# jdeschut/tunempc

Measured on AMD Instinct MI355X. Metric: stage-Hessian convexifications/sec at (nx+nu)=32, p=64, higher is better.
Workload: dtype f64

## Files before the change

### tunempc_amd/csrc/tmpc_persist.h

```cpp
#pragma once
#include "tmpc_common.h"
#include "tmpc_cr_small.h"
#include "tmpc_factor.h"
#include "tmpc_schur.h"
#include "tmpc_stage.h"

namespace tmpc {

constexpr int PK_NMAX = sm8::NMAX;
constexpr int PK_WAVE_DOUBLES = 6 * sm8::MS + 16;
static_assert(PK_WAVE_DOUBLES >= sm8::MS + 160, "step-length scratch");
static_assert(PK_WAVE_DOUBLES >= 25 * 10 + 16, "records of schur_body<0> at nx = 5");
constexpr int pk_lds_doubles(int p) {
  int v = CRS_NW * PK_WAVE_DOUBLES;
  if (crs_factor_lds_doubles() > v) v = crs_factor_lds_doubles();
  if (crs_solve_lds_doubles(p) > v) v = crs_solve_lds_doubles(p);
  return v;
}

__global__ void __launch_bounds__(CRS_NT) k_ipm_small(WS w, Dims dm, Opts o, CrDev cr, CrLevs lv, int prep, int reg_max, double chord_pre, int cap) {
  extern __shared__ __attribute__((aligned(16))) double lds[];
  const int b = w.alist ? w.alist[blockIdx.x] : (int)blockIdx.x;
  const int tid = threadIdx.x, lane = tid & 63, wv = tid >> 6;
  double* smw = lds + wv * PK_WAVE_DOUBLES;
  const int p = dm.p, s0 = b * p;
  volatile int* ip = w.iprob + (size_t)b * IS;
#ifdef TMPC_CYCLE_PROF
  unsigned long long tpk_ = __builtin_readcyclecounter();
#define PK_T(i) { __syncthreads(); if (blockIdx.x == 0 && threadIdx.x == 0) { const unsigned long long t_ = __builtin_readcyclecounter(); g_prof[48 + (i)] += t_ - tpk_; tpk_ = t_; } }
#else
#define PK_T(i) __syncthreads();
#endif
  for (int it = 0; it < cap; ++it) {
    if (ip[I_PHASE] == PH_DONE) break;
    for (int k = wv; k < p; k += CRS_NW) sm8::stage_pre_body<64>(w, dm, s0 + k, lane, smw);
    PK_T(0)
    if (wv == 0) ctrl_a_body(w, dm, o, b, lane);
    PK_T(1)
    const int phase = ip[I_PHASE];
    if (phase == PH_DONE) break;
    if (!ip[I_CHORD]) {
      for (int k = wv; k < p; k += CRS_NW) {
        schur_body<0, false, 64>(w, dm, s0 + k, lane, smw);
        schur_body<1, false, 64>(w, dm, s0 + k, lane, smw);
      }
      PK_T(2)
      if (prep) { cr_prep_body<CRS_NT>(w, dm, b, prep); __syncthreads(); }
      cr_small_factor_body(w, dm, cr, lv, b, lds);
      PK_T(3)
    }
    for (int pass = 1; pass <= 2; ++pass) {
      if (pass == 2 || phase == PH_MAIN) {
        for (int k = wv; k < p; k += CRS_NW) sm8::stage_rhs_body<64>(w, dm, s0 + k, lane, smw, pass);
        PK_T(4)
        for (int k = wv; k < p; k += CRS_NW) gather_body(w, dm, s0 + k, lane, pass);
        PK_T(5)
        cr_small_solve_body(w, dm, cr, lv, b, lds, pass);
        PK_T(6)
        solve_border_body<CRS_NT>(w, dm, b, pass, lds);
        PK_T(7)
        for (int k = wv; k < p; k += CRS_NW) sm8::stage_dir_body<64>(w, dm, s0 + k, lane, smw, pass);
        PK_T(8)
        for (int m = tid; m < 4 * p; m += CRS_NT) eigmin_lane_body(w, dm, 4 * s0 + m, pass);
        PK_T(9)
      }
      if (wv == 0) { if (pass == 1) ctrl_b_body(w, dm, reg_max, b, lane); else ctrl_c_body(w, dm, reg_max, b, lane); }
      PK_T(10)
    }
    for (int k = wv; k < p; k += CRS_NW) sm8::update_body<64>(w, dm, s0 + k, lane);
    __syncthreads();
    if (tid == 0) ctrl_d_body(w, dm, o, b, false);
    PK_T(11)
  }
#undef PK_T
}

}
```

### tunempc_amd/csrc/tmpc_stage.h

```cpp
#pragma once
#include "tmpc_common.h"
#include "tmpc_small.h"

namespace tmpc {

__device__ __forceinline__ int stage_id4(const WS& w, const Dims& dm) {
  if (!w.alist) return blockIdx.x;
  const int sb = blockIdx.x >> 2, bi = sb / dm.p;
  return ((w.alist[bi] * dm.p + (sb - bi * dm.p)) << 2) | (blockIdx.x & 3);
}

#define TMPC_STAGE_PROLOGUE                                     \
  const int sid = stage_id(w, dm);                              \
  const int b = sid / dm.p;                                     \
  const int k = sid - b * dm.p;                                 \
  const int lane = threadIdx.x;                                 \
  const int n = dm.n, nx = dm.nx;                               \
  const int nn = n * n, nxx = nx * nx;                          \
  (void)k; (void)nn; (void)nxx;                                 \
  extern __shared__ __attribute__((aligned(16))) double sm[];

#ifdef TMPC_EIG_DEBUG
__device__ int g_eig_dbg[4]; __device__ double g_eig_dbgv[8];
#endif

__device__ __forceinline__ int stage_rows(const WS& w, const Dims& dm, size_t sid) {
  int nc = w.ncnt ? w.ncnt[sid] : 0;
  nc = nc < 0 ? 0 : (nc > dm.nr - dm.ng ? dm.nr - dm.ng : nc);
  return dm.ng + nc;
}

#include "tmpc_stage_impl.h"
namespace sm8 {
#include "tmpc_stage_impl.h"
}

__global__ void __launch_bounds__(64) k_init_stage(WS w, Dims dm) {
  TMPC_STAGE_PROLOGUE
  double* sH = sm; double* cs = sm + MS;
  const double* Hg = w.H + (size_t)sid * nn;
  for (int e = lane; e < nn; e += 64) {
    int i, j; ediv(e, n, i, j);
    sH[i * LD + j] = 0.5 * (Hg[i * n + j] + Hg[j * n + i]);
  }
  wsync();
  s2g(w.Hb + (size_t)sid * nn, sH, n, n, n, lane);
  jacobi_eigvals(sH, n, cs, lane);
  double lo = 1e300, hi = -1e300, amin = 1e300, amax = 0.0;
  if (lane < n) {
    const double ev = sH[lane * LD + lane];
    lo = ev; hi = ev;
    const double a = fabs(ev);
    if (a != 0.0) { amin = a; amax = a; }
  }
  lo = wave_min(lo); hi = wave_max(hi); amin = wave_min(amin); amax = wave_max(amax);
  if (lane == 0) {
    double* q = w.part + (size_t)sid * NPART;
    q[Q_MINEIG] = lo; q[Q_MAXEIG] = hi; q[Q_MINABS] = amin; q[Q_MAXABS] = amax;
  }
  const int mb = dm.mb;
  double* Vg = w.V + (size_t)sid * nx * n;
  const double* Ag = w.A + (size_t)sid * nxx;
  const double* Bg = w.Bm + (size_t)sid * nx * mb;
  for (int e = lane; e < nx * n; e += 64) {
    int i, j; ediv(e, n, i, j);
    Vg[e] = (j < nx) ? Ag[i * nx + j] : Bg[i * mb + (j - nx)];
  }
}

__global__ void __launch_bounds__(64) k_init_prob(WS w, Dims dm, double lowp_switch) {
  const int b = blockIdx.x, lane = threadIdx.x;
  double lo = 1e300, amin = 1e10 , amax = 0.0;
  for (int k = lane; k < dm.p; k += 64) {
    const double* q = w.part + (size_t)(b * dm.p + k) * NPART;
    lo = fmin(lo, q[Q_MINEIG]); amin = fmin(amin, q[Q_MINABS]); amax = fmax(amax, q[Q_MAXABS]);
  }
  lo = wave_min(lo); amin = wave_min(amin); amax = wave_max(amax);
  if (lane == 0) {
    double* pr = w.prob + (size_t)b * PS;
    int* ip = w.iprob + (size_t)b * IS;
    for (int i = 0; i < PS; ++i) pr[i] = 0.0;
    for (int i = 0; i < IS; ++i) ip[i] = 0;
    const double s = 1.0 / amin, sbeta = amax / amin;
    pr[P_S] = s; pr[P_SBETA] = sbeta; pr[P_MINEIG_H] = lo;
    pr[P_TAU] = 2.0; pr[P_ALPHA] = 1.0 / sbeta; pr[P_S0] = 1.0 / sbeta; pr[P_X0] = 1.0 / (double)(dm.p * dm.n);
    pr[P_MUT] = -1.0; pr[P_PREVSTEPN] = -1.0; pr[P_STEPN] = 1e300; pr[P_MINPIV] = 1.0;
    const int early = (lo > 0.0) ? 1 : 0;
    ip[I_EARLY] = early;
    ip[I_PHASE] = early ? PH_DONE : PH_MAIN;
    ip[I_IPMSTATUS] = early ? IPM_OPTIMAL : IPM_MAXITER;
    if (!early) { const int slot = atomicAdd(w.active, 1); w.alist[slot] = b; w.flist[slot] = b; }
    if (!early && (dm.flags & DF_LOWP) && w.O32 && 2.0 / (double)(2 * dm.p * dm.n + 1) > lowp_switch * fmax(1.0, fabs(pr[P_TAU]))) { ip[I_LOWP] = 1; atomicAdd(w.active + 4, 1); }
  }
}

__global__ void __launch_bounds__(64) k_init_state(WS w, Dims dm) {
  TMPC_STAGE_PROLOGUE
  const double* pr = w.prob + (size_t)b * PS;
  const double s = pr[P_S], tau = pr[P_TAU], alpha = pr[P_ALPHA];
  const double x0 = 1.0 / (double)(dm.p * n);
  double* Hb = w.Hb + (size_t)sid * nn;
  for (int e = lane; e < nn; e += 64) {
    int i, j; ediv(e, n, i, j);
    const double hb = s * Hb[e];
    Hb[e] = hb;
    const double dg = (i == j) ? 1.0 : 0.0;
    w.S1[(size_t)sid * nn + e] = dg;
    w.S2[(size_t)sid * nn + e] = tau * dg - alpha * hb;
    w.X1[(size_t)sid * nn + e] = x0 * dg;
    w.X2[(size_t)sid * nn + e] = x0 * dg;
  }
  for (int e = lane; e < nxx; e += 64) w.P[(size_t)sid * nxx + e] = 0.0;
}

__device__ __forceinline__ double lane_min_eig8(const double* __restrict__ Wg, int n) {
  double a[36];
#define TMPC_A8(i, j) a[(i) * ((i) + 1) / 2 + (j)]
#define TMPC_S8(r, c) (((c) <= (r)) ? TMPC_A8(r, c) : TMPC_A8(c, r))
#pragma unroll
  for (int i = 0; i < 8; ++i)
#pragma unroll
    for (int j = 0; j <= i; ++j) TMPC_A8(i, j) = (i < n) ? 0.5 * (Wg[i * n + j] + Wg[j * n + i]) : 0.0;
#pragma unroll
  for (int j = 0; j < 6; ++j) {
    double sigma = 0.0;
#pragma unroll
    for (int i = j + 2; i < 8; ++i) sigma = fma(TMPC_A8(i, j), TMPC_A8(i, j), sigma);
    if (sigma != 0.0) {
      const double x0 = TMPC_A8(j + 1, j);
      const double mu = sqrt(fma(x0, x0, sigma));
      const double v0 = (x0 <= 0.0) ? (x0 - mu) : (-sigma / (x0 + mu));
      const double beta = 2.0 * v0 * v0 / (sigma + v0 * v0);
      const double rv0 = 1.0 / v0;
      double v[8], pw[8];
#pragma unroll
      for (int i = j + 1; i < 8; ++i) v[i] = (i == j + 1) ? 1.0 : TMPC_A8(i, j) * rv0;
      double kk = 0.0;
#pragma unroll
      for (int r = j + 1; r < 8; ++r) {
        double acc = 0.0;
#pragma unroll
        for (int c = j + 1; c < 8; ++c) acc = fma(TMPC_S8(r, c), v[c], acc);
        pw[r] = beta * acc;
        kk = fma(pw[r], v[r], kk);
      }
      kk *= 0.5 * beta;
#pragma unroll
      for (int r = j + 1; r < 8; ++r) pw[r] = fma(-kk, v[r], pw[r]);
#pragma unroll
      for (int r = j + 1; r < 8; ++r)
#pragma unroll
        for (int c = j + 1; c <= r; ++c) TMPC_A8(r, c) -= fma(v[r], pw[c], pw[r] * v[c]);
      TMPC_A8(j + 1, j) = mu;
    }
  }
  double dd[8], ee[8];
#pragma unroll
  for (int i = 0; i < 8; ++i) { dd[i] = TMPC_A8(i, i); ee[i] = (i < 7) ? TMPC_A8(i + 1, i) : 0.0; }
#undef TMPC_S8
#undef TMPC_A8
  if (n == 1) return dd[0];
  double scale = 0.0;
  bool bad = false;
#pragma unroll
  for (int i = 0; i < 8; ++i) if (i < n) { bad |= !(dd[i] == dd[i]) || ((i + 1 < n) && !(ee[i] == ee[i])); scale = fmax(scale, fmax(fabs(dd[i]), (i + 1 < n) ? fabs(ee[i]) : 0.0)); }
  if (bad) return __builtin_nan("");
  if (!(scale > 0.0) || !(scale < 1e300)) return (scale == 0.0) ? 0.0 : scale;
  const double rs = 1.0 / scale;
  double e2[8];
  double lo = 1e300;
#pragma unroll
  for (int i = 0; i < 8; ++i) {
    dd[i] *= rs; ee[i] *= rs; e2[i] = ee[i] * ee[i];
  }
#pragma unroll
  for (int i = 0; i < 8; ++i)
    if (i < n) lo = fmin(lo, dd[i] - ((i > 0) ? fabs(ee[i - 1]) : 0.0) - ((i + 1 < n) ? fabs(ee[i]) : 0.0));
  double x = lo - 1e-14;
  const double dn = (double)n;
  for (int it = 0; it < 64; ++it) {
    double qm = 1.0, q = dd[0] - x, gm = 0.0, g = -1.0, hm = 0.0, h = 0.0;
#pragma unroll
    for (int i = 1; i < 8; ++i) {
      if (i < n) {
        const double t = dd[i] - x, c = e2[i - 1];
        const double qn = fma(t, q, -c * qm);
        const double gn = fma(t, g, -c * gm) - q;
        const double hn = fma(t, h, -c * hm) - 2.0 * g;
        qm = q; q = qn; gm = g; g = gn; hm = h; h = hn;
      }
    }
    if (!(q > 0.0)) break;
    const double G = g / q, H = G * G - h / q;
    double disc = (dn - 1.0) * (dn * H - G * G);
    if (!(disc > 0.0)) disc = 0.0;
    const double step = dn / (sqrt(disc) - G);
    if (!(step > 4e-16 * fmax(1.0, fabs(x)))) break;
    x += step;
  }
  return x * scale;
}
__device__ __forceinline__ void eigmin_lane_body(const WS& w, const Dims& dm, int mid, int pass) {
  const int b = (mid >> 2) / dm.p;
  const int phase = w.iprob[(size_t)b * IS + I_PHASE];
  if (phase == PH_DONE || (pass == 1 && phase != PH_MAIN)) return;
  w.eigmin[mid] = lane_min_eig8(w.Wm + (size_t)mid * dm.n * dm.n, dm.n);
}
__global__ void __launch_bounds__(64) k_eigmin_lane(WS w, Dims dm, int pass, int nmat) {
  const int i = blockIdx.x * 64 + threadIdx.x;
  if (i >= nmat) return;
  const int sb = i >> 2, bi = sb / dm.p;
  const int mid = w.alist ? (((w.alist[bi] * dm.p + (sb - bi * dm.p)) << 2) | (i & 3)) : i;
  eigmin_lane_body(w, dm, mid, pass);
}

template <int NT>
__global__ void __launch_bounds__(NT, NT == 256 ? 3 : 1) k_stage_pre(WS w, Dims dm) {
  extern __shared__ __attribute__((aligned(16))) double sm[];
  stage_pre_body<NT>(w, dm, stage_id(w, dm), threadIdx.x, sm);
}
template <int NT>
__global__ void __launch_bounds__(NT, NT == 256 ? 3 : 1) k_stage_rhs(WS w, Dims dm, int pass) {
  extern __shared__ __attribute__((aligned(16))) double sm[];
  stage_rhs_body<NT>(w, dm, stage_id(w, dm), threadIdx.x, sm, pass);
}
template <int NT>
__global__ void __launch_bounds__(NT, NT == 256 ? 3 : 1) k_stage_dir(WS w, Dims dm, int pass) {
  extern __shared__ __attribute__((aligned(16))) double sm[];
  stage_dir_body<NT>(w, dm, stage_id(w, dm), threadIdx.x, sm, pass);
}
__global__ void __launch_bounds__(64) k_eigmin(WS w, Dims dm, int pass, double chord_step) {
  extern __shared__ __attribute__((aligned(16))) double sm[];
  eigmin_body(w, dm, stage_id4(w, dm), threadIdx.x, sm, pass, chord_step);
}
template <int NT>
__global__ void __launch_bounds__(NT) k_update(WS w, Dims dm) {
  update_body<NT>(w, dm, stage_id(w, dm), threadIdx.x);
}

constexpr int FIN_SLOTS = 6;
__global__ void __launch_bounds__(64) k_final_stage(WS w, Dims dm) {
  TMPC_STAGE_PROLOGUE
  const int* ip = w.iprob + (size_t)b * IS;
  const double* pr = w.prob + (size_t)b * PS;
  double* sV = sm; double* sM = sm + MS; double* t0 = sm + 2 * MS; double* t1 = sm + 3 * MS; double* sHb = sm + 4 * MS;
  double* cs = sm + 5 * MS;
  const int kn = (k + 1 == dm.p) ? 0 : k + 1;
  const double sc = ip[I_EARLY] ? 0.0 : 1.0 / (pr[P_S] * pr[P_ALPHA]);
  double* Po = w.Pout + (size_t)sid * nxx;
  for (int e = lane; e < nxx; e += 64) Po[e] = sc * w.P[(size_t)sid * nxx + e];
  double* Pon = w.Pout + (size_t)(b * dm.p + kn) * nxx;
  const double* Pn = w.P + (size_t)(b * dm.p + kn) * nxx;
  if (kn != k) { for (int e = lane; e < nxx; e += 64) Pon[e] = sc * Pn[e]; }
  __threadfence_block();
  wsync();
  g2s(sV, w.V + (size_t)sid * nx * n, nx, n, n, lane);
  const double* Hg = w.H + (size_t)sid * nn;
  for (int e = lane; e < nn; e += 64) { int i, j; ediv(e, n, i, j); sHb[i * LD + j] = 0.5 * (Hg[i * n + j] + Hg[j * n + i]); }
  wsync();
  build_M(sM, sV, t0, t1, sHb, Po, Pon, 0.0, n, nx, lane);
  if (dm.nr > 0) {
    const int nrow = stage_rows(w, dm, sid);
    if (lane < dm.nr) w.Fg[(size_t)sid * dm.nr + lane] = (lane < nrow) ? sc * w.phi[(size_t)sid * dm.nr + lane] : 0.0;
    add_gtg(sM, w.G + (size_t)sid * dm.nr * n, w.phi + (size_t)sid * dm.nr, sc, nrow, n, lane);
  }
  if (dm.nT > 0) {
    add_smat_t3(sM, w.t3th + (size_t)sid * dm.nT, sc, n, lane);
    for (int e = lane; e < nn; e += 64) {
      int i, j; ediv(e, n, i, j);
      const int a = i < j ? i : j, bq = i < j ? j : i;
      w.Tout[(size_t)sid * nn + e] = sc * w.t3th[(size_t)sid * dm.nT + a * n - a * (a - 1) / 2 + (bq - a)];
    }
  }
  s_sym(sM, n, lane);
  double* dHg = w.dHc + (size_t)sid * nn;
  double* Hcg = w.Hc + (size_t)sid * nn;
  for (int e = lane; e < nn; e += 64) {
    int i, j; ediv(e, n, i, j);
    const double dh = sM[i * LD + j];
    dHg[e] = dh;
    const double hc = sHb[i * LD + j] + dh;
    Hcg[e] = hc;
    t0[i * LD + j] = hc;
  }
  wsync();
  const double lo = tridiag_min_eig(t0, n, cs, lane);
  const double hi = tridiag_max_after(cs, n, lane);
  if (lane == 0) {
    double* q = w.part + (size_t)sid * NPART;
    q[Q_MINEIG] = lo; q[Q_MAXEIG] = hi;
  }
}

__global__ void __launch_bounds__(64) k_final_prob(WS w, Dims dm) {
  const int b = blockIdx.x, lane = threadIdx.x;
  double lo = 1e300, hi = -1e300, mc = 0.0;
  for (int k = lane; k < dm.p; k += 64) {
    const double* q = w.part + (size_t)(b * dm.p + k) * NPART;
    lo = fmin(lo, q[Q_MINEIG]); hi = fmax(hi, q[Q_MAXEIG]);
    mc = fmax(mc, (q[Q_MINEIG] > 0.0) ? q[Q_MAXEIG] / q[Q_MINEIG] : 1e300);
  }
  lo = wave_min(lo); hi = wave_max(hi); mc = wave_max(mc);
  if (lane == 0) {
    double* pr = w.prob + (size_t)b * PS;
    int* ip = w.iprob + (size_t)b * IS;
    pr[P_MINEIG_HC] = lo; pr[P_MAXEIG_HC] = hi; pr[P_MAXCOND] = mc;
    int st;
    if (lo > 0.0) st = (ip[I_IPMSTATUS] == IPM_OPTIMAL || ip[I_IPMSTATUS] == IPM_FAST_EXIT || ip[I_IPMSTATUS] == IPM_TIGHT_FALLBACK) ? ST_OPTIMAL : ST_FEASIBLE;
    else st = ST_INFEASIBLE;
    ip[I_STATUS] = st;
    if (ip[I_EARLY]) { pr[P_KAPPA] = 0.0; pr[P_BETA] = 0.0; pr[P_ALPHA_OUT] = 1.0; }
    else { pr[P_KAPPA] = pr[P_TAU]; pr[P_BETA] = pr[P_TAU] / pr[P_SBETA]; pr[P_ALPHA_OUT] = pr[P_ALPHA]; }
  }
}

}
```

### tunempc_amd/csrc/tmpc_stage_impl.h

```cpp
template <int NT = 64>
__device__ __forceinline__ void s2g_T(double* g, const double* s, int rows, int cols, int ldg, int lane) {
  const int tot = rows * cols;
  for (int e = lane; e < tot; e += NT) {
    const int j = e / rows, i = e - j * rows;
    g[(size_t)j * ldg + i] = s[i * LD + j];
  }
  wsync();
}

template <int NT = 64>
__device__ __forceinline__ void build_M(double* out, const double* sV, double* t0, double* t1, const double* sHb,
                                        const double* Pk, const double* Pn, double coef, int n, int nx, int lane) {
  g2s<NT>(t0, Pn, nx, nx, nx, lane);
  mm<NT>(t1, sV, 1, LD, t0, LD, 1, n, nx, nx, 0, lane);
  mm<NT>(out, t1, LD, 1, sV, LD, 1, n, n, nx, 0, lane);
  g2s<NT>(t0, Pk, nx, nx, nx, lane);
  for (int e = lane; e < n * n; e += NT) {
    int i, j; ediv(e, n, i, j);
    double v = out[i * LD + j] + coef * sHb[i * LD + j];
    if (i < nx && j < nx) v -= t0[i * LD + j];
    out[i * LD + j] = v;
  }
  wsync();
}

template <int NT = 64>
__device__ __forceinline__ void adj_V(double* out, double* t, const double* sV, const double* G, int n, int nx, int lane) {
  mm<NT>(t, sV, LD, 1, G, LD, 1, nx, n, n, 0, lane);
  mm<NT>(out, t, LD, 1, sV, 1, LD, nx, nx, n, 0, lane);
}

template <int NT = 64>
__device__ __forceinline__ void add_gtg(double* out, const double* Gg, const double* coef, double scale, int ng, int n, int lane) {
  for (int e = lane; e < n * n; e += NT) {
    int i, j; ediv(e, n, i, j);
    double acc = 0.0;
    for (int r = 0; r < ng; ++r) acc = fma(scale * coef[r] * Gg[r * n + i], Gg[r * n + j], acc);
    out[i * LD + j] += acc;
  }
  wsync();
}

template <int NT = 64>
__device__ __forceinline__ void add_smat_t3(double* out, const double* th, double scale, int n, int lane) {
  for (int e = lane; e < n * n; e += NT) {
    int i, j; ediv(e, n, i, j);
    const int a = i < j ? i : j, b = i < j ? j : i;
    out[i * LD + j] += scale * th[a * n - a * (a - 1) / 2 + (b - a)];
  }
  wsync();
}

constexpr int PRE_SLOTS = 6;
template <int NT>
__device__ __forceinline__ void stage_pre_body(const WS& w, const Dims& dm, int sid, int lane, double* sm) {
  const int b = sid / dm.p;
  const int k = sid - b * dm.p;
  const int n = dm.n, nx = dm.nx;
  const int nn = n * n, nxx = nx * nx;
  (void)k; (void)nn; (void)nxx;
  const int* ip = w.iprob + (size_t)b * IS;
  if (ip[I_PHASE] == PH_DONE) return;
  const double* pr = w.prob + (size_t)b * PS;
  const double alpha = pr[P_ALPHA], tau = pr[P_TAU];
  double* sV = sm; double* sX = sm + MS; double* sS = sm + 2 * MS; double* t0 = sm + 3 * MS; double* t1 = sm + 4 * MS; double* sLi = sm + 5 * MS;
  double* sHb = sX;
  double* sM = sS;
  double* sSi = sS;
  double* t2 = sLi;
  double* sPhi = sX;
  constexpr int EPT = NMAX * NMAX / NT;
  double hbr[EPT], phir[EPT];
  const int kn = (k + 1 == dm.p) ? 0 : k + 1;
  TMPC_T0()
  double ldA[EPT];
  g2r<NT>(ldA, w.V + (size_t)sid * nx * n, nx, n, n, lane);
  g2r<NT>(hbr, w.Hb + (size_t)sid * nn, n, n, n, lane);
  r2s<NT>(sV, ldA, nx, n, lane);
  r2s<NT>(sHb, hbr, n, n, lane);
  TMPC_T(8)
#pragma unroll
  for (int q = 0; q < EPT; ++q) phir[q] = 0.0;
  build_M<NT>(sM, sV, t0, t1, sHb, w.P + (size_t)sid * nxx, w.P + (size_t)(b * dm.p + kn) * nxx, alpha, n, nx, lane);
  if (dm.nr > 0) add_gtg<NT>(sM, w.G + (size_t)sid * dm.nr * n, w.phi + (size_t)sid * dm.nr, 1.0, stage_rows(w, dm, sid), n, lane);
  if (dm.nT > 0) add_smat_t3<NT>(sM, w.t3th + (size_t)sid * dm.nT, 1.0, n, lane);
  TMPC_T(9)
  double rd2 = 0.0, s2 = 0.0, xs = 0.0, trx2 = 0.0, hby = 0.0, trpsi = 0.0, trphi2 = 0.0;
  int nbad = 0;
  double* kf = w.KF + (size_t)sid * 12 * nxx;
  for (int r = 0; r < 2; ++r) {
    const double* Sg = (r ? w.S2 : w.S1) + (size_t)sid * nn;
    double* Rdg = (r ? w.Rd2 : w.Rd1) + (size_t)sid * nn;
    for (int e = lane; e < nn; e += NT) {
      int i, j; ediv(e, n, i, j);
      const double m = sM[i * LD + j], sv = Sg[e];
      const double dg = (i == j) ? 1.0 : 0.0;
      const double rd = (r == 0 ? (m - dg) : (tau * dg - m)) - sv;
      Rdg[e] = rd;
      rd2 = fma(rd, rd, rd2); s2 = fma(sv, sv, s2);
    }
  }
  wsync();
  TMPC_T(10)
  for (int r = 0; r < 2; ++r) {
    const double* Xg = (r ? w.X2 : w.X1) + (size_t)sid * nn;
    const double* Sg = (r ? w.S2 : w.S1) + (size_t)sid * nn;
    {
      double ldB[EPT];
      g2r<NT>(ldA, Xg, n, n, n, lane);
      g2r<NT>(ldB, Sg, n, n, n, lane);
      r2s<NT>(sX, ldA, n, n, lane);
      r2s<NT>(sS, ldB, n, n, lane);
    }
    TMPC_T(8)
    for (int e = lane; e < nn; e += NT) { int i, j; ediv(e, n, i, j); xs = fma(sX[i * LD + j], sS[i * LD + j], xs); }
    {
      double hx = 0.0;
#pragma unroll
      for (int q = 0; q < EPT; ++q) { const int e = lane + q * NT; int i, j; ediv(e, n, i, j); if (e < nn) hx = fma(hbr[q], sX[i * LD + j], hx); }
      hx = block_sum<NT>(hx);
      if (r == 0) hby += hx; else { hby -= hx; trx2 = trace_s<NT>(sX, n, lane); }
    }
    for (int e = lane; e < nn; e += NT) { int i, j; ediv(e, n, i, j); t0[i * LD + j] = sX[i * LD + j]; }
    wsync();
    TMPC_T(10)
    if (NT == 256 && n == 32 && NMAX >= 32) {
      nbad += chol_inv_pair32<NT>(sS, sLi, t0, t1, lane);
      TMPC_T(11)
    } else {
      nbad += chol_lower_pair_t<NT>(sS, t0, n, lane);
      TMPC_T(11)
      tri_inv_lower_pair_t<NT>(sLi, sS, t1, t0, n, lane);
    }
    TMPC_T(12)
    s2g<NT>((r ? w.L2i : w.L1i) + (size_t)sid * nn, sLi, n, n, n, lane);
    s2g<NT>((r ? w.LX2i : w.LX1i) + (size_t)sid * nn, t1, n, n, n, lane);
    TMPC_T(13)
    mm<NT>(sSi, sLi, 1, LD, sLi, LD, 1, n, n, n, 0, lane);
    TMPC_T(14)
    s_sym<NT>(sSi, n, lane);
    s2g<NT>((r ? w.S2i : w.S1i) + (size_t)sid * nn, sSi, n, n, n, lane);
    TMPC_T(13)
    double* kfr = kf + (size_t)r * KF_PER_LMI * nxx;
    mm<NT>(t0, sV, LD, 1, sX, LD, 1, nx, n, n, 0, lane);
    mm<NT>(t1, t0, LD, 1, sV, 1, LD, nx, nx, n, 0, lane);
    s2g<NT>(kfr + KF_KX * nxx, t1, nx, nx, nx, lane);
    s2g_T<NT>(kfr + KF_FX * nxx, t0, nx, nx, nx, lane);
    s2g<NT>(kfr + KF_XXX * nxx, sX, nx, nx, nx, lane);
    mm<NT>(t0, sV, LD, 1, sSi, LD, 1, nx, n, n, 0, lane);
    mm<NT>(t1, t0, LD, 1, sV, 1, LD, nx, nx, n, 0, lane);
    s2g<NT>(kfr + KF_KS * nxx, t1, nx, nx, nx, lane);
    s2g_T<NT>(kfr + KF_FS * nxx, t0, nx, nx, nx, lane);
    s2g<NT>(kfr + KF_SIXX * nxx, sSi, nx, nx, nx, lane);
    r2s<NT>(t1, hbr, n, n, lane);
    mm<NT>(t0, sX, LD, 1, t1, LD, 1, n, n, n, 0, lane);
    mm<NT>(t1, t0, LD, 1, sSi, LD, 1, n, n, n, 0, lane);
#pragma unroll
    for (int q = 0; q < EPT; ++q) {
      const int e = lane + q * NT;
      if (e < nn) {
        int i, j; ediv(e, n, i, j);
        const double phi = 0.5 * (t1[i * LD + j] + t1[j * LD + i]);
        phir[q] += phi;
        if (r == 1 && i == j) trphi2 += phi;
      }
    }
    wsync();
    if (r == 1) {
      mm<NT>(t0, sX, LD, 1, sSi, LD, 1, n, n, n, 0, lane);
      s_sym<NT>(t0, n, lane);
      trpsi = trace_s<NT>(t0, n, lane);
      if (dm.nT > 0) s2g<NT>(w.t3psi + (size_t)sid * nn, t0, n, n, n, lane);
      adj_V<NT>(t1, t2, sV, t0, n, nx, lane);
      s2g<NT>(w.adjV + ((size_t)sid * NADJ + ADJ_PSI) * nxx, t1, nx, nx, nx, lane);
      s2g<NT>(w.adjE + ((size_t)sid * NADJ + ADJ_PSI) * nxx, t0, nx, nx, nx, lane);
    }
  }
  TMPC_T(15)
  double hbphi = 0.0;
#pragma unroll
  for (int q = 0; q < EPT; ++q) {
    const int e = lane + q * NT;
    if (e < nn) { int i, j; ediv(e, n, i, j); sPhi[i * LD + j] = phir[q]; hbphi = fma(hbr[q], phir[q], hbphi); }
  }
  wsync();
  hbphi = block_sum<NT>(hbphi);
  if (dm.nT > 0) s2g<NT>(w.t3phi + (size_t)sid * nn, sPhi, n, n, n, lane);
  adj_V<NT>(t1, t2, sV, sPhi, n, nx, lane);
  s2g<NT>(w.adjV + ((size_t)sid * NADJ + ADJ_PHI) * nxx, t1, nx, nx, nx, lane);
  s2g<NT>(w.adjE + ((size_t)sid * NADJ + ADJ_PHI) * nxx, sPhi, nx, nx, nx, lane);
  rd2 = block_sum<NT>(rd2); s2 = block_sum<NT>(s2); xs = block_sum<NT>(xs); trphi2 = block_sum<NT>(trphi2);
  if (lane == 0) {
    double* q = w.part + (size_t)sid * NPART;
    q[Q_XS] = xs; q[Q_RD2] = rd2; q[Q_S2] = s2; q[Q_TRX2] = trx2; q[Q_HBY] = hby;
    q[Q_TRPSI] = trpsi; q[Q_TRPHI2] = trphi2; q[Q_HBPHI] = hbphi; q[Q_CHOLBAD] = (double)nbad;
  }
}

constexpr int RHS_SLOTS = 6;
template <int NT>
__device__ __forceinline__ void stage_rhs_body(const WS& w, const Dims& dm, int sid, int lane, double* sm, int pass) {
  const int b = sid / dm.p;
  const int k = sid - b * dm.p;
  const int n = dm.n, nx = dm.nx;
  const int nn = n * n, nxx = nx * nx;
  (void)k; (void)nn; (void)nxx;
  const int* ip = w.iprob + (size_t)b * IS;
  const int phase = ip[I_PHASE];
  if (phase == PH_DONE || (pass == 1 && phase != PH_MAIN)) return;
  const double* pr = w.prob + (size_t)b * PS;
  const double sig = (pass == 1) ? 0.0 : pr[P_SIGMU];
  const bool use_corr = (pass == 2 && phase == PH_MAIN);
  double* sV = sm; double* sX = sm + MS; double* sSi = sm + 2 * MS; double* sRd = sm + 3 * MS;
  double* t0 = sm + 4 * MS; double* t1 = sm + 5 * MS;
  double* sG = sRd;
  constexpr int EPT = NMAX * NMAX / NT;
  double gr[EPT];
#pragma unroll
  for (int q = 0; q < EPT; ++q) gr[q] = 0.0;
  g2s<NT>(sV, w.V + (size_t)sid * nx * n, nx, n, n, lane);
  double trt2 = 0.0;
  for (int r = 0; r < 2; ++r) {
    {
      double l0[EPT], l1[EPT], l2[EPT];
      g2r<NT>(l0, (r ? w.X2 : w.X1) + (size_t)sid * nn, n, n, n, lane);
      g2r<NT>(l1, (r ? w.S2i : w.S1i) + (size_t)sid * nn, n, n, n, lane);
      g2r<NT>(l2, (r ? w.Rd2 : w.Rd1) + (size_t)sid * nn, n, n, n, lane);
      r2s<NT>(sX, l0, n, n, lane); r2s<NT>(sSi, l1, n, n, lane); r2s<NT>(sRd, l2, n, n, lane);
    }
    mm<NT>(t0, sX, LD, 1, sRd, LD, 1, n, n, n, 0, lane);
    mm<NT>(t1, t0, LD, 1, sSi, LD, 1, n, n, n, 0, lane);
    double* Tg = (r ? w.T2 : w.T1) + (size_t)sid * nn;
    const double* cg = (r ? w.c2 : w.c1) + (size_t)sid * nn;
#pragma unroll
    for (int q = 0; q < EPT; ++q) {
      const int e = lane + q * NT;
      if (e < nn) {
        int i, j; ediv(e, n, i, j);
        double t = sig * sSi[i * LD + j] - 0.5 * (t1[i * LD + j] + t1[j * LD + i]);
        if (use_corr) t -= cg[e];
        Tg[e] = t;
        if (r == 0) gr[q] = t; else { gr[q] -= t; if (i == j) trt2 += t; }
      }
    }
    wsync();
  }
  double hbg = 0.0;
  {
    const double* Hbg = w.Hb + (size_t)sid * nn;
#pragma unroll
    for (int q = 0; q < EPT; ++q) {
      const int e = lane + q * NT;
      if (e < nn) { int i, j; ediv(e, n, i, j); sG[i * LD + j] = gr[q]; hbg = fma(Hbg[e], gr[q], hbg); }
    }
  }
  wsync();
  hbg = block_sum<NT>(hbg);
  adj_V<NT>(t1, t0, sV, sG, n, nx, lane);
  s2g<NT>(w.adjV + ((size_t)sid * NADJ + ADJ_G) * nxx, t1, nx, nx, nx, lane);
  s2g<NT>(w.adjE + ((size_t)sid * NADJ + ADJ_G) * nxx, sG, nx, nx, nx, lane);
  trt2 = block_sum<NT>(trt2);
  if (lane == 0) {
    double* q = w.part + (size_t)sid * NPART;
    q[Q_TRT2] = trt2; q[Q_HBG] = hbg;
  }
}

constexpr int DIR_SLOTS = 6;
template <int NT>
__device__ __forceinline__ void stage_dir_body(const WS& w, const Dims& dm, int sid, int lane, double* sm, int pass) {
  const int b = sid / dm.p;
  const int k = sid - b * dm.p;
  const int n = dm.n, nx = dm.nx;
  const int nn = n * n, nxx = nx * nx;
  (void)k; (void)nn; (void)nxx;
  const int* ip = w.iprob + (size_t)b * IS;
  const int phase = ip[I_PHASE];
  if (phase == PH_DONE || (pass == 1 && phase != PH_MAIN)) return;
  const double* pr = w.prob + (size_t)b * PS;
  const double dtau = pr[P_DTAU], dalpha = pr[P_DALPHA];
  double* sX = sm; double* sSi = sm + MS; double* sDS = sm + 2 * MS; double* sDX = sm + 3 * MS; double* t0 = sm + 4 * MS; double* t1 = sm + 5 * MS;
  double* sV = sX; double* sHb = sSi; double* sM = sDS;
  double* sL = sX;
  constexpr int EPT = NMAX * NMAX / NT;
  double dmr[EPT];
  const int kn = (k + 1 == dm.p) ? 0 : k + 1;
  {
    double l0[EPT], l1[EPT];
    g2r<NT>(l0, w.V + (size_t)sid * nx * n, nx, n, n, lane);
    g2r<NT>(l1, w.Hb + (size_t)sid * nn, n, n, n, lane);
    r2s<NT>(sV, l0, nx, n, lane); r2s<NT>(sHb, l1, n, n, lane);
  }
  const double* dPk = w.dP + (size_t)sid * nxx;
  build_M<NT>(sM, sV, t0, t1, sHb, dPk, w.dP + (size_t)(b * dm.p + kn) * nxx, dalpha, n, nx, lane);
  if (dm.nr > 0) add_gtg<NT>(sM, w.G + (size_t)sid * dm.nr * n, w.dphi + (size_t)sid * dm.nr, 1.0, stage_rows(w, dm, sid), n, lane);
  if (dm.nT > 0) add_smat_t3<NT>(sM, w.t3dth + (size_t)sid * dm.nT, 1.0, n, lane);
#pragma unroll
  for (int q = 0; q < EPT; ++q) { const int e = lane + q * NT; int i, j; ediv(e, n, i, j); dmr[q] = (e < nn) ? sM[i * LD + j] : 0.0; }
  wsync();
  double dxs = 0.0, xds = 0.0, dxds = 0.0;
  for (int r = 0; r < 2; ++r) {
    const double* Xg = (r ? w.X2 : w.X1) + (size_t)sid * nn;
    const double* Sg = (r ? w.S2 : w.S1) + (size_t)sid * nn;
    const double* Rdg = (r ? w.Rd2 : w.Rd1) + (size_t)sid * nn;
    const double* Tg = (r ? w.T2 : w.T1) + (size_t)sid * nn;
    double* dSg = (r ? w.dS2 : w.dS1) + (size_t)sid * nn;
    double* dXg = (r ? w.dX2 : w.dX1) + (size_t)sid * nn;
    double lL[EPT], lLX[EPT];
    {
      double l0[EPT], l1[EPT];
      g2r<NT>(l0, Xg, n, n, n, lane);
      g2r<NT>(l1, (r ? w.S2i : w.S1i) + (size_t)sid * nn, n, n, n, lane);
      g2r<NT>(lL, (r ? w.L2i : w.L1i) + (size_t)sid * nn, n, n, n, lane);
      g2r<NT>(lLX, (r ? w.LX2i : w.LX1i) + (size_t)sid * nn, n, n, n, lane);
      r2s<NT>(sX, l0, n, n, lane); r2s<NT>(sSi, l1, n, n, lane);
    }
#pragma unroll
    for (int q = 0; q < EPT; ++q) {
      const int e = lane + q * NT;
      if (e < nn) {
        int i, j; ediv(e, n, i, j);
        const double dm_ = dmr[q];
        const double ldy = (r == 0) ? dm_ : ((i == j ? dtau : 0.0) - dm_);
        sDX[i * LD + j] = ldy;
        const double ds = ldy + Rdg[e];
        sDS[i * LD + j] = ds;
        dSg[e] = ds;
      }
    }
    wsync();
    mm<NT>(t0, sX, LD, 1, sDX, LD, 1, n, n, n, 0, lane);
    mm<NT>(t1, t0, LD, 1, sSi, LD, 1, n, n, n, 0, lane);
    for (int e = lane; e < nn; e += NT) {
      int i, j; ediv(e, n, i, j);
      const double dx = Tg[e] - sX[i * LD + j] - 0.5 * (t1[i * LD + j] + t1[j * LD + i]);
      sDX[i * LD + j] = dx;
      dXg[e] = dx;
      const double ds = sDS[i * LD + j];
      dxs = fma(dx, Sg[e], dxs); xds = fma(sX[i * LD + j], ds, xds); dxds = fma(dx, ds, dxds);
    }
    wsync();
    r2s<NT>(sL, lL, n, n, lane);
    mm<NT>(t0, sL, LD, 1, sDS, LD, 1, n, n, n, 0, lane);
    mm<NT>(t1, t0, LD, 1, sL, 1, LD, n, n, n, 0, lane);
    s2g_sym<NT>(w.Wm + ((size_t)sid * 4 + 2 * r) * nn, t1, n, lane);
    r2s<NT>(sL, lLX, n, n, lane);
    mm<NT>(t0, sL, LD, 1, sDX, LD, 1, n, n, n, 0, lane);
    mm<NT>(t1, t0, LD, 1, sL, 1, LD, n, n, n, 0, lane);
    s2g_sym<NT>(w.Wm + ((size_t)sid * 4 + 2 * r + 1) * nn, t1, n, lane);
    if (pass == 1) {
      mm<NT>(t0, sDX, LD, 1, sDS, LD, 1, n, n, n, 0, lane);
      mm<NT>(t1, t0, LD, 1, sSi, LD, 1, n, n, n, 0, lane);
      s2g_sym<NT>((r ? w.c2 : w.c1) + (size_t)sid * nn, t1, n, lane);
    }
  }
  double dh2 = 0.0, m2 = 0.0;
  {
    const double ra = dalpha / pr[P_ALPHA];
    const double* S1g = w.S1 + (size_t)sid * nn; const double* R1g = w.Rd1 + (size_t)sid * nn;
#pragma unroll
    for (int q = 0; q < EPT; ++q) {
      const int e = lane + q * NT;
      if (e < nn) {
        int i, j; ediv(e, n, i, j);
        const double m = S1g[e] + R1g[e] + (i == j ? 1.0 : 0.0);
        const double dh = dmr[q] - ra * m;
        dh2 = fma(dh, dh, dh2); m2 = fma(m, m, m2);
      }
    }
    dh2 = block_sum<NT>(dh2); m2 = block_sum<NT>(m2);
  }
  double dp2 = 0.0, p2 = 0.0;
  const double* Pk = w.P + (size_t)sid * nxx;
  for (int e = lane; e < nxx; e += NT) { dp2 = fma(dPk[e], dPk[e], dp2); p2 = fma(Pk[e], Pk[e], p2); }
  dxs = block_sum<NT>(dxs); xds = block_sum<NT>(xds); dxds = block_sum<NT>(dxds); dp2 = block_sum<NT>(dp2); p2 = block_sum<NT>(p2);
  if (lane == 0) {
    double* q = w.part + (size_t)sid * NPART;
    q[Q_DXS] = dxs; q[Q_XDS] = xds; q[Q_DXDS] = dxds; q[Q_DP2] = dp2; q[Q_P2] = p2; q[Q_DH2] = dh2; q[Q_M2] = m2;
  }
}

__device__ __forceinline__ void eigmin_body(const WS& w, const Dims& dm, int mid, int lane, double* sm, int pass, double chord_step) {
  const int b = (mid >> 2) / dm.p;
  const int* ip = w.iprob + (size_t)b * IS;
  const int phase = ip[I_PHASE];
  if (phase == PH_DONE || (pass == 1 && phase != PH_MAIN)) return;
  const int n = dm.n;
  double* A = sm;
  double* cs = A + MS;
  const double* Wg = w.Wm + (size_t)mid * n * n;
  TMPC_TC0()
  g2s(A, Wg, n, n, n, lane);
  TMPC_TC(5, 0)
  double th[2]; int nth = 0;
  if (chord_step < 0.0) {}
  else if (pass == 1) {}
  else if (phase == PH_MAIN) th[nth++] = (1.0 / 0.9) * (1.0 + 1e-9);
  else {
    if (chord_step > 1.0 / TMPC_CENTER_DAMP) th[nth++] = chord_step * (1.0 + 1e-9);
    th[nth++] = (1.0 / TMPC_CENTER_DAMP) * (1.0 + 1e-9);
  }
  for (int t = 0; t < nth; ++t) {
    if (shifted_is_pd(A, th[t], n, lane)) {
#ifdef TMPC_EIG_DEBUG
      wsync(); g2s(A, Wg, n, n, n, lane);
      const double ex = tridiag_min_eig(A, n, cs, lane);
      if (lane == 0) { atomicAdd(&g_eig_dbg[0], 1); if (ex <= -1.0 / th[t]) { if (atomicAdd(&g_eig_dbg[1], 1) == 0) { g_eig_dbgv[0] = ex; g_eig_dbgv[1] = th[t]; g_eig_dbgv[2] = pass; g_eig_dbgv[3] = phase; } } }
#endif
      if (lane == 0) w.eigmin[mid] = -1.0 / th[t];
      return;
    }
    wsync();
    g2s(A, Wg, n, n, n, lane);
#ifdef TMPC_EIG_DEBUG
    { const double ex = tridiag_min_eig(A, n, cs, lane);
      if (lane == 0) { atomicAdd(&g_eig_dbg[2], 1); if (ex > -1.0 / th[t]) { if (atomicAdd(&g_eig_dbg[3], 1) == 0) { g_eig_dbgv[4] = ex; g_eig_dbgv[5] = th[t]; g_eig_dbgv[6] = pass; g_eig_dbgv[7] = phase; } } }
      wsync(); g2s(A, Wg, n, n, n, lane); }
#endif
  }
  const double lo = tridiag_min_eig(A, n, cs, lane);
  TMPC_TC(5, 3)
  if (lane == 0) w.eigmin[mid] = lo;
}

template <int NT>
__device__ __forceinline__ void update_body(const WS& w, const Dims& dm, int sid, int lane) {
  const int b = sid / dm.p;
  const int n = dm.n, nx = dm.nx;
  const int nn = n * n, nxx = nx * nx;
  const int* ip = w.iprob + (size_t)b * IS;
  if (ip[I_PHASE] == PH_DONE) return;
  const double* pr = w.prob + (size_t)b * PS;
  const double ap = pr[P_AP], ad = pr[P_AD];
  if (ap == 0.0 && ad == 0.0) return;
  const size_t o = (size_t)sid * nn;
  for (int e = lane; e < nn; e += NT) {
    int i, j; ediv(e, n, i, j);
    const int et = j * n + i;
    if (j <= i) {
      const double x1 = 0.5 * ((w.X1[o + e] + ap * w.dX1[o + e]) + (w.X1[o + et] + ap * w.dX1[o + et]));
      const double x2 = 0.5 * ((w.X2[o + e] + ap * w.dX2[o + e]) + (w.X2[o + et] + ap * w.dX2[o + et]));
      const double s1 = 0.5 * ((w.S1[o + e] + ad * w.dS1[o + e]) + (w.S1[o + et] + ad * w.dS1[o + et]));
      const double s2 = 0.5 * ((w.S2[o + e] + ad * w.dS2[o + e]) + (w.S2[o + et] + ad * w.dS2[o + et]));
      w.X1[o + e] = x1; w.X1[o + et] = x1; w.X2[o + e] = x2; w.X2[o + et] = x2;
      w.S1[o + e] = s1; w.S1[o + et] = s1; w.S2[o + e] = s2; w.S2[o + et] = s2;
    }
  }
  for (int e = lane; e < nxx; e += NT) w.P[(size_t)sid * nxx + e] += ad * w.dP[(size_t)sid * nxx + e];
}
```

Measured before the change: 12490.

## Shrink LDS scratch in stage rhs/dir bodies by aliasing buffers

Reworks the shared-memory scratch layout of the stage RHS and direction bodies. RHS drops from six slots to three and DIR from six to four by reusing buffers in place, keeping Hb in registers, and reordering the pass-1 c computation. The persistent kernel's per-wave scratch is sized from the largest slot count, and the RHS kernel's launch-bounds occupancy hint rises from 3 to 7. The goal is lower LDS use and higher occupancy, at the cost of relying on in-place matmuls being safe and of extra register pressure.

```diff
diff --git a/tunempc_amd/csrc/tmpc_persist.h b/tunempc_amd/csrc/tmpc_persist.h
--- a/tunempc_amd/csrc/tmpc_persist.h
+++ b/tunempc_amd/csrc/tmpc_persist.h
@@ -8,7 +8,9 @@
 namespace tmpc {
 
 constexpr int PK_NMAX = sm8::NMAX;
-constexpr int PK_WAVE_DOUBLES = 6 * sm8::MS + 16;
+constexpr int PK_STAGE_SLOTS = sm8::PRE_SLOTS > sm8::DIR_SLOTS ? (sm8::PRE_SLOTS > sm8::RHS_SLOTS ? sm8::PRE_SLOTS : sm8::RHS_SLOTS)
+                                                               : (sm8::DIR_SLOTS > sm8::RHS_SLOTS ? sm8::DIR_SLOTS : sm8::RHS_SLOTS);
+constexpr int PK_WAVE_DOUBLES = PK_STAGE_SLOTS * sm8::MS + 16;
 static_assert(PK_WAVE_DOUBLES >= sm8::MS + 160, "step-length scratch");
 static_assert(PK_WAVE_DOUBLES >= 25 * 10 + 16, "records of schur_body<0> at nx = 5");
 constexpr int pk_lds_doubles(int p) {
diff --git a/tunempc_amd/csrc/tmpc_stage.h b/tunempc_amd/csrc/tmpc_stage.h
--- a/tunempc_amd/csrc/tmpc_stage.h
+++ b/tunempc_amd/csrc/tmpc_stage.h
@@ -220,7 +220,7 @@
   stage_pre_body<NT>(w, dm, stage_id(w, dm), threadIdx.x, sm);
 }
 template <int NT>
-__global__ void __launch_bounds__(NT, NT == 256 ? 3 : 1) k_stage_rhs(WS w, Dims dm, int pass) {
+__global__ void __launch_bounds__(NT, NT == 256 ? 7 : 1) k_stage_rhs(WS w, Dims dm, int pass) {
   extern __shared__ __attribute__((aligned(16))) double sm[];
   stage_rhs_body<NT>(w, dm, stage_id(w, dm), threadIdx.x, sm, pass);
 }
diff --git a/tunempc_amd/csrc/tmpc_stage_impl.h b/tunempc_amd/csrc/tmpc_stage_impl.h
--- a/tunempc_amd/csrc/tmpc_stage_impl.h
+++ b/tunempc_amd/csrc/tmpc_stage_impl.h
@@ -20,6 +20,26 @@
     double v = out[i * LD + j] + coef * sHb[i * LD + j];
     if (i < nx && j < nx) v -= t0[i * LD + j];
     out[i * LD + j] = v;
+  }
+  wsync();
+}
+
+template <int NT>
+__device__ __forceinline__ void build_M_r(double* out, const double* sV, double* t0, double* t1, const double (&hbr)[NMAX * NMAX / NT],
+                                          const double* Pk, const double* Pn, double coef, int n, int nx, int lane) {
+  g2s<NT>(t0, Pn, nx, nx, nx, lane);
+  mm<NT>(t1, sV, 1, LD, t0, LD, 1, n, nx, nx, 0, lane);
+  mm<NT>(out, t1, LD, 1, sV, LD, 1, n, n, nx, 0, lane);
+  g2s<NT>(t0, Pk, nx, nx, nx, lane);
+#pragma unroll
+  for (int q = 0; q < NMAX * NMAX / NT; ++q) {
+    const int e = lane + q * NT;
+    if (e < n * n) {
+      int i, j; ediv(e, n, i, j);
+      double v = out[i * LD + j] + coef * hbr[q];
+      if (i < nx && j < nx) v -= t0[i * LD + j];
+      out[i * LD + j] = v;
+    }
   }
   wsync();
 }
@@ -197,7 +217,7 @@
   }
 }
 
-constexpr int RHS_SLOTS = 6;
+constexpr int RHS_SLOTS = 3;
 template <int NT>
 __device__ __forceinline__ void stage_rhs_body(const WS& w, const Dims& dm, int sid, int lane, double* sm, int pass) {
   const int b = sid / dm.p;
@@ -211,14 +231,15 @@
   const double* pr = w.prob + (size_t)b * PS;
   const double sig = (pass == 1) ? 0.0 : pr[P_SIGMU];
   const bool use_corr = (pass == 2 && phase == PH_MAIN);
-  double* sV = sm; double* sX = sm + MS; double* sSi = sm + 2 * MS; double* sRd = sm + 3 * MS;
-  double* t0 = sm + 4 * MS; double* t1 = sm + 5 * MS;
+  double* sX = sm; double* sSi = sm + MS; double* sRd = sm + 2 * MS;
+  double* t1 = sRd;
+  double* sV = sX;
   double* sG = sRd;
+  double* tA = sSi;
   constexpr int EPT = NMAX * NMAX / NT;
   double gr[EPT];
 #pragma unroll
   for (int q = 0; q < EPT; ++q) gr[q] = 0.0;
-  g2s<NT>(sV, w.V + (size_t)sid * nx * n, nx, n, n, lane);
   double trt2 = 0.0;
   for (int r = 0; r < 2; ++r) {
     {
@@ -228,8 +249,8 @@
       g2r<NT>(l2, (r ? w.Rd2 : w.Rd1) + (size_t)sid * nn, n, n, n, lane);
       r2s<NT>(sX, l0, n, n, lane); r2s<NT>(sSi, l1, n, n, lane); r2s<NT>(sRd, l2, n, n, lane);
     }
-    mm<NT>(t0, sX, LD, 1, sRd, LD, 1, n, n, n, 0, lane);
-    mm<NT>(t1, t0, LD, 1, sSi, LD, 1, n, n, n, 0, lane);
+    mm<NT>(sRd, sX, LD, 1, sRd, LD, 1, n, n, n, 0, lane);
+    mm<NT>(t1, sRd, LD, 1, sSi, LD, 1, n, n, n, 0, lane);
     double* Tg = (r ? w.T2 : w.T1) + (size_t)sid * nn;
     const double* cg = (r ? w.c2 : w.c1) + (size_t)sid * nn;
 #pragma unroll
@@ -254,10 +275,10 @@
       if (e < nn) { int i, j; ediv(e, n, i, j); sG[i * LD + j] = gr[q]; hbg = fma(Hbg[e], gr[q], hbg); }
     }
   }
-  wsync();
+  g2s<NT>(sV, w.V + (size_t)sid * nx * n, nx, n, n, lane);
   hbg = block_sum<NT>(hbg);
-  adj_V<NT>(t1, t0, sV, sG, n, nx, lane);
-  s2g<NT>(w.adjV + ((size_t)sid * NADJ + ADJ_G) * nxx, t1, nx, nx, nx, lane);
+  adj_V<NT>(tA, tA, sV, sG, n, nx, lane);
+  s2g<NT>(w.adjV + ((size_t)sid * NADJ + ADJ_G) * nxx, tA, nx, nx, nx, lane);
   s2g<NT>(w.adjE + ((size_t)sid * NADJ + ADJ_G) * nxx, sG, nx, nx, nx, lane);
   trt2 = block_sum<NT>(trt2);
   if (lane == 0) {
@@ -266,7 +287,7 @@
   }
 }
 
-constexpr int DIR_SLOTS = 6;
+constexpr int DIR_SLOTS = 4;
 template <int NT>
 __device__ __forceinline__ void stage_dir_body(const WS& w, const Dims& dm, int sid, int lane, double* sm, int pass) {
   const int b = sid / dm.p;
@@ -279,20 +300,21 @@
   if (phase == PH_DONE || (pass == 1 && phase != PH_MAIN)) return;
   const double* pr = w.prob + (size_t)b * PS;
   const double dtau = pr[P_DTAU], dalpha = pr[P_DALPHA];
-  double* sX = sm; double* sSi = sm + MS; double* sDS = sm + 2 * MS; double* sDX = sm + 3 * MS; double* t0 = sm + 4 * MS; double* t1 = sm + 5 * MS;
-  double* sV = sX; double* sHb = sSi; double* sM = sDS;
-  double* sL = sX;
+  double* sX = sm; double* sSi = sm + MS; double* sDS = sm + 2 * MS; double* sDX = sm + 3 * MS;
+  double* sV = sX; double* sM = sDX;
+  double* sW = sX;
+  double* sL = sSi;
   constexpr int EPT = NMAX * NMAX / NT;
   double dmr[EPT];
   const int kn = (k + 1 == dm.p) ? 0 : k + 1;
+  const double* dPk = w.dP + (size_t)sid * nxx;
   {
-    double l0[EPT], l1[EPT];
+    double l0[EPT], hbr[EPT];
     g2r<NT>(l0, w.V + (size_t)sid * nx * n, nx, n, n, lane);
-    g2r<NT>(l1, w.Hb + (size_t)sid * nn, n, n, n, lane);
-    r2s<NT>(sV, l0, nx, n, lane); r2s<NT>(sHb, l1, n, n, lane);
-  }
-  const double* dPk = w.dP + (size_t)sid * nxx;
-  build_M<NT>(sM, sV, t0, t1, sHb, dPk, w.dP + (size_t)(b * dm.p + kn) * nxx, dalpha, n, nx, lane);
+    g2r<NT>(hbr, w.Hb + (size_t)sid * nn, n, n, n, lane);
+    r2s<NT>(sV, l0, nx, n, lane);
+    build_M_r<NT>(sM, sV, sSi, sDS, hbr, dPk, w.dP + (size_t)(b * dm.p + kn) * nxx, dalpha, n, nx, lane);
+  }
   if (dm.nr > 0) add_gtg<NT>(sM, w.G + (size_t)sid * dm.nr * n, w.dphi + (size_t)sid * dm.nr, 1.0, stage_rows(w, dm, sid), n, lane);
   if (dm.nT > 0) add_smat_t3<NT>(sM, w.t3dth + (size_t)sid * dm.nT, 1.0, n, lane);
 #pragma unroll
@@ -329,30 +351,46 @@
       }
     }
     wsync();
-    mm<NT>(t0, sX, LD, 1, sDX, LD, 1, n, n, n, 0, lane);
-    mm<NT>(t1, t0, LD, 1, sSi, LD, 1, n, n, n, 0, lane);
-    for (int e = lane; e < nn; e += NT) {
-      int i, j; ediv(e, n, i, j);
-      const double dx = Tg[e] - sX[i * LD + j] - 0.5 * (t1[i * LD + j] + t1[j * LD + i]);
-      sDX[i * LD + j] = dx;
-      dXg[e] = dx;
-      const double ds = sDS[i * LD + j];
-      dxs = fma(dx, Sg[e], dxs); xds = fma(sX[i * LD + j], ds, xds); dxds = fma(dx, ds, dxds);
-    }
-    wsync();
+    mm<NT>(sDX, sX, LD, 1, sDX, LD, 1, n, n, n, 0, lane);
+    mm<NT>(sDX, sDX, LD, 1, sSi, LD, 1, n, n, n, 0, lane);
+    {
+      double dxr[EPT];
+#pragma unroll
+      for (int q = 0; q < EPT; ++q) {
+        const int e = lane + q * NT;
+        if (e < nn) {
+          int i, j; ediv(e, n, i, j);
+          dxr[q] = Tg[e] - sX[i * LD + j] - 0.5 * (sDX[i * LD + j] + sDX[j * LD + i]);
+        }
+      }
+      wsync();
+#pragma unroll
+      for (int q = 0; q < EPT; ++q) {
+        const int e = lane + q * NT;
+        if (e < nn) {
+          int i, j; ediv(e, n, i, j);
+          const double dx = dxr[q];
+          sDX[i * LD + j] = dx;
+          dXg[e] = dx;
+          const double ds = sDS[i * LD + j];
+          dxs = fma(dx, Sg[e], dxs); xds = fma(sX[i * LD + j], ds, xds); dxds = fma(dx, ds, dxds);
+        }
+      }
+    }
+    wsync();
+    if (pass == 1) {
+      mm<NT>(sW, sDX, LD, 1, sDS, LD, 1, n, n, n, 0, lane);
+      mm<NT>(sW, sW, LD, 1, sSi, LD, 1, n, n, n, 0, lane);
+      s2g_sym<NT>((r ? w.c2 : w.c1) + (size_t)sid * nn, sW, n, lane);
+    }
     r2s<NT>(sL, lL, n, n, lane);
-    mm<NT>(t0, sL, LD, 1, sDS, LD, 1, n, n, n, 0, lane);
-    mm<NT>(t1, t0, LD, 1, sL, 1, LD, n, n, n, 0, lane);
-    s2g_sym<NT>(w.Wm + ((size_t)sid * 4 + 2 * r) * nn, t1, n, lane);
+    mm<NT>(sW, sL, LD, 1, sDS, LD, 1, n, n, n, 0, lane);
+    mm<NT>(sW, sW, LD, 1, sL, 1, LD, n, n, n, 0, lane);
+    s2g_sym<NT>(w.Wm + ((size_t)sid * 4 + 2 * r) * nn, sW, n, lane);
     r2s<NT>(sL, lLX, n, n, lane);
-    mm<NT>(t0, sL, LD, 1, sDX, LD, 1, n, n, n, 0, lane);
-    mm<NT>(t1, t0, LD, 1, sL, 1, LD, n, n, n, 0, lane);
-    s2g_sym<NT>(w.Wm + ((size_t)sid * 4 + 2 * r + 1) * nn, t1, n, lane);
-    if (pass == 1) {
-      mm<NT>(t0, sDX, LD, 1, sDS, LD, 1, n, n, n, 0, lane);
-      mm<NT>(t1, t0, LD, 1, sSi, LD, 1, n, n, n, 0, lane);
-      s2g_sym<NT>((r ? w.c2 : w.c1) + (size_t)sid * nn, t1, n, lane);
-    }
+    mm<NT>(sW, sL, LD, 1, sDX, LD, 1, n, n, n, 0, lane);
+    mm<NT>(sW, sW, LD, 1, sL, 1, LD, n, n, n, 0, lane);
+    s2g_sym<NT>(w.Wm + ((size_t)sid * 4 + 2 * r + 1) * nn, sW, n, lane);
   }
   double dh2 = 0.0, m2 = 0.0;
   {
```

Result: no change. 12600 (median of 6 runs) (+0.8%).
